# cloudflare/flow-pipeline

Measured on AMD Instinct MI355X. Metric: FlowMessages/sec aggregated into flows_5m, higher is better.
Workload: dtype u64

## Files before the change

### flow-pipeline_amd/csrc/agg.cuh

```cuda
#pragma once
#include <hip/hip_runtime.h>
#include <stdint.h>

#include "sinks.cuh"

namespace fa {

struct AggTable {
    unsigned long long k0[AGG_SLOTS], k1[AGG_SLOTS], s1[AGG_SLOTS], s2[AGG_SLOTS];
};
static_assert(sizeof(AggTable) == 32 * AGG_SLOTS, "agg_kernel LDS table");

__device__ __forceinline__ bool agg_lds_upsert(AggTable& lt, uint64_t k0, uint64_t k1, uint32_t h, uint32_t by,
                                               unsigned long long v2) {
    uint32_t i = h & (AGG_SLOTS - 1);
#pragma unroll 1
    for (int probe = 0; probe < AGG_PROBES; probe++, i = (i + 1) & (AGG_SLOTS - 1)) {
        unsigned long long c0 = lt.k0[i];
        if (c0 == 0) c0 = atomicCAS(&lt.k0[i], 0ull, (unsigned long long)k0);
        if (c0 != 0 && c0 != k0) continue;
        unsigned long long c1 = lt.k1[i];
        if (c1 == 0) c1 = atomicCAS(&lt.k1[i], 0ull, (unsigned long long)k1);
        if (c1 != 0 && c1 != k1) continue;
        if (by) atomicAdd(&lt.s1[i], (unsigned long long)by);
// ... 101 lines not shown
            if (qn + cnt > 64u) {
                agg_drain(a, lt, tb_base, lane, queue, qn);
                qn = 0;
            }
            if (pnd)
                queue[qn + (uint32_t)__builtin_popcountll(m & ((1ull << lane) - 1ull))] =
                    tup16_pack(tv[s].src_as, tv[s].dst_as, tv[s].bytes, tv[s].packets, tv[s].tbr, tv[s].etype);
            qn += cnt;
        }
    }
}

__device__ __forceinline__ void agg_consume(const KArgs& a, AggTable& lt, uint32_t tb_base, uint32_t lane, const AggBatch& b, uint4* queue,
                                            uint32_t& qn) {
    constexpr int NT = AGG_SU;
    static_assert(NT % AGG_CH == 0, "batch = whole chunks");
    agg_consume_chunk<0>(a, lt, tb_base, lane, b, queue, qn);
    if constexpr (NT > AGG_CH) agg_consume_chunk<AGG_CH>(a, lt, tb_base, lane, b, queue, qn);
    if constexpr (NT > 2 * AGG_CH) agg_consume_chunk<2 * AGG_CH>(a, lt, tb_base, lane, b, queue, qn);
    if constexpr (NT > 3 * AGG_CH) agg_consume_chunk<3 * AGG_CH>(a, lt, tb_base, lane, b, queue, qn);
    static_assert(NT <= 4 * AGG_CH, "agg_consume: add chunks");
}

__global__ __launch_bounds__(AGG_BLOCK) void agg_kernel(KArgs a) {
    __shared__ AggTable lt;
    __shared__ uint32_t pc[AGG_MAX_NWG + AGG_PAD];
    const uint32_t part = blockIdx.x;
    for (int i = threadIdx.x; i < AGG_SLOTS; i += AGG_BLOCK) {
        lt.k0[i] = 0;
        lt.k1[i] = 0;
        lt.s1[i] = 0;
        lt.s2[i] = 0;
    }
    __shared__ uint32_t pcb[AGG_MAX_NWG + AGG_PAD];
    __shared__ uint4 queues[(AGG_BLOCK / 64) * 64];
    __shared__ uint32_t maxc_s[2];
    if (threadIdx.x < 3) maxc_s[threadIdx.x] = 0;
    __syncthreads();
    uint32_t mymax = 0, mymaxb = 0, mysum = 0;
    for (uint32_t i = threadIdx.x; i < AGG_MAX_NWG + AGG_PAD; i += AGG_BLOCK) {
        const uint32_t c = i < a.nwg ? a.seg_counts[(size_t)part * a.nwg + i] : 0u;
        const uint32_t cb = i < a.nwg ? a.seg_counts[((size_t)NPART_MAX + part) * a.nwg + i] : 0u;
        pc[i] = c;
        pcb[i] = cb;
        mymax = max(mymax, c);
        mymaxb = max(mymaxb, cb);
        mysum += c + cb;
    }
    for (int o = 32; o > 0; o >>= 1) {
        mymax = max(mymax, (uint32_t)__shfl_xor((int)mymax, o));
        mymaxb = max(mymaxb, (uint32_t)__shfl_xor((int)mymaxb, o));
        mysum += (uint32_t)__shfl_xor((int)mysum, o);
    }
    if ((threadIdx.x & 63) == 0) {
        atomicMax(&maxc_s[0], mymax);
        atomicMax(&maxc_s[1], mymaxb);
        if (mysum) atomicAdd(&maxc_s[2], mysum);
    }
    const uint32_t tb_base = a.ctr->tb_base;
// ... 42 lines not shown
    ulonglong2 home[NF];
    uint32_t fh[NF];
#pragma unroll
    for (int q = 0; q < NF; q++) {
        const int i = q * AGG_BLOCK + threadIdx.x;
        fk0[q] = lt.k0[i];
        fk1[q] = lt.k1[i];
        fs1[q] = lt.s1[i];
        fs2[q] = lt.s2[i];
        fh[q] = key_hash(fk0[q], fk1[q]);
        home[q] = *reinterpret_cast<const ulonglong2*>(&a.tab[as_home(fk0[q], fk1[q], fh[q], a.mask, a.rlog2)]);
    }
#pragma unroll
    for (int q = 0; q < NF; q++) {
        Slot* sp = nullptr;
        const unsigned long long b = fs1[q], p = fs2[q] >> 25, c = fs2[q] & 0x1ffffffull;
        if (fk0[q] != 0 && fk1[q] != 0 && fs2[q] != 0) {
            if (home[q].x == fk0[q] && home[q].y == fk1[q]) sp = &a.tab[as_home(fk0[q], fk1[q], fh[q], a.mask, a.rlog2)];
            else sp = table_find_or_claim(a, fk0[q], fk1[q], fh[q]);
            if (!sp) spill_park(a, fk0[q], fk1[q], b, p, c);
        }
        quad_atomic_update(sp, b, p, c);
    }
}

constexpr int AGG8_SLOTS = 4096;
constexpr int AGG8_ALL = AGG8_SLOTS + AGG_PROBES;
struct Agg8Table {
    unsigned long long key[AGG8_ALL], s1[AGG8_ALL], s2[AGG8_ALL];
};
__device__ __forceinline__ unsigned long long agg8_key(const uint2& t) { return (1ull << 63) | ((unsigned long long)(t.y >> 26) << 32) | t.x; }
__device__ __forceinline__ uint32_t agg8_mix(const uint2& t) { return (t.x ^ ((t.y >> 26) * 0x9E3779B1u)) * 0x85EBCA6Bu; }
__device__ __forceinline__ uint32_t agg8_home(const uint2& t) {
    return agg8_mix(t) >> 20;
}
__device__ __forceinline__ uint32_t agg8_sub(const uint2& t) { return (agg8_mix(t) >> 17) & 7u; }
__device__ __forceinline__ void agg8_global(const KArgs& a, uint32_t tb_base, uint32_t part, const uint2& t, uint32_t by, uint32_t pk) {
    TupleVals v;
    t8_unpack(t, part, tb_base, v);
    uint64_t k0, k1;
    pack_key(tb_base + v.tbr, v.src_as, v.dst_as, v.etype, k0, k1);
    agg_global(a, k0, k1, key_hash(k0, k1), by, pk, 1);
}
__device__ __forceinline__ void agg8_tuple(const KArgs& a, Agg8Table& lt, uint32_t tb_base, uint32_t part, const uint2& t) {
    const unsigned long long key = agg8_key(t);
    const uint32_t by = t.y & 0x1ffffu, pk = (t.y >> 17) & 0x1ffu;
// ... 68 lines not shown
        b.v |= valid << (2 * s);
        idx[s] = valid ? piece : 0u;
    }
#pragma unroll
    for (int s = 0; s < SU; s++) b.t[s] = pbase[(size_t)min(seg[s], nwg - 1u) * (capq / 2u) + idx[s]];
}
__device__ __forceinline__ void agg8_drain(const KArgs& a, Agg8Table& lt, uint32_t tb_base, uint32_t part, uint32_t lane, const uint2* queue, uint32_t qn) {
    if (lane < qn) agg8_tuple(a, lt, tb_base, part, queue[lane]);
}
__device__ __forceinline__ unsigned long long agg8_find_heavy(unsigned long long key, bool valid) {
    unsigned long long rest = __builtin_amdgcn_ballot_w64(valid);
#pragma unroll 1
    for (int attempt = 0; attempt < 2 && rest != 0ull; attempt++) {
        const int l = __builtin_ctzll(rest);
        const unsigned long long k = readlane_u64(key, l);
        const unsigned long long same = __builtin_amdgcn_ballot_w64(valid && key == k);
        if (__builtin_popcountll(same) >= 8) return k;
        rest &= ~same;
    }
    return 0ull;
}
__device__ __forceinline__ void agg8_consume(const KArgs& a, Agg8Table& lt, uint32_t tb_base, uint32_t part, uint32_t lane, const Agg8Batch& b,
                                             uint2* queue, uint32_t& qn, uint32_t pmask, uint32_t pass, unsigned long long& hk) {
    uint2 t[AGG8_NT];
    unsigned long long key[AGG8_NT], c0[AGG8_NT], c1[AGG8_NT];
    uint32_t home[AGG8_NT];
#pragma unroll
    for (int e = 0; e < AGG8_NT; e++) {
        const uint4& q = b.t[e >> 1];
        t[e] = (e & 1) ? make_uint2(q.z, q.w) : make_uint2(q.x, q.y);
        key[e] = agg8_key(t[e]);
        home[e] = agg8_home(t[e]);
        c0[e] = lt.key[home[e]];
        c1[e] = lt.key[home[e] + 1];
    }
    if (FA_DBG(a, DBG_AGG_NO_LDS)) {
        unsigned long long x = 0;
#pragma unroll
        for (int e = 0; e < AGG8_NT; e++) x ^= c0[e] ^ c1[e] ^ key[e];
        if (x == 0x12345678ull) lt.s1[lane] = x;
        return;
    }
    uint32_t pending = 0;
    if (hk < 4ull) {
        const unsigned long long f = agg8_find_heavy(key[0], (b.v & 1u) && !(pmask && (agg8_sub(t[0]) & pmask) != pass));
        hk = f ? f : hk + 1ull;
// ... 109 lines not shown
            while (g < ngroups && j >= (uint32_t)__builtin_amdgcn_readfirstlane((int)LV[min(g, (uint32_t)(NG) - 1u)])) { \
                g += WAVES;                                                                                 \
                j = 0;                                                                                      \
            }                                                                                               \
        };                                                                                                  \
        settle_item();                                                                                      \
        Agg8Batch b0, b1;                                                                                   \
        agg8_fetch<BACK, AGG8_SU>(a.capq, a.nwg, pbase, PCNT, g * (GSEGS), lane, j, b0);                                          \
        while (g < ngroups) {                                                                               \
            j++;                                                                                            \
            settle_item();                                                                                  \
            agg8_fetch<BACK, AGG8_SU>(a.capq, a.nwg, pbase, PCNT, g * (GSEGS), lane, j, b1);                                      \
            agg8_consume(a, lt, tb_base, part, lane, b0, queue, qn, pmask, pass, hk);                                       \
            if (g >= ngroups) break;                                                                        \
            j++;                                                                                            \
            settle_item();                                                                                  \
            agg8_fetch<BACK, AGG8_SU>(a.capq, a.nwg, pbase, PCNT, g * (GSEGS), lane, j, b0);                                      \
            agg8_consume(a, lt, tb_base, part, lane, b1, queue, qn, pmask, pass, hk);                                       \
        }                                                                                                   \
    }
    FA_AGG8_PASS(false, flv, NFG, FGRP, pc)
    FA_AGG8_PASS(true, blv, NBG, BGRP, pcb)
#undef FA_AGG8_PASS
    agg8_drain(a, lt, tb_base, part, lane, queue, qn);
    __syncthreads();
    const unsigned long long tm1 = (FA_DBG(a, DBG_TIMING | DBG_AGG8_TIMING)) ? (FA_DBG(a, DBG_AGG8_TIMING) ? wall_clock64() : clock64()) : 0ull;
    if (FA_DBG(a, DBG_AGG_NO_FLUSH)) return;
    constexpr int NF = (AGG8_ALL + AGG_BLOCK - 1) / AGG_BLOCK, FB = 3;
    auto group_of = [&](int i, uint64_t& k0, uint64_t& k1, unsigned long long& s1, unsigned long long& s2) -> bool {
        const unsigned long long key = i < AGG8_ALL ? lt.key[i] : 0ull;
        s1 = i < AGG8_ALL ? lt.s1[i] : 0ull;
        s2 = i < AGG8_ALL ? lt.s2[i] : 0ull;
        TupleVals v;
        t8_unpack(make_uint2((uint32_t)key, (uint32_t)(key >> 32) << 26), part, tb_base, v);
        pack_key(tb_base + v.tbr, v.src_as, v.dst_as, v.etype, k0, k1);
        return key != 0ull && s2 != 0ull;
    };
    if (a.rlog2 == AS_RLOG2_MAX && !(a.dbg & DBG_AGG_ATOMIC_FLUSH)) {
        const uint32_t rmask = a.mask >> AS_RLOG2_MAX;
#pragma unroll 1
        for (int q0 = 0; q0 < NF; q0 += FB) {
            uint64_t fk0[FB], fk1[FB];
            unsigned long long fs1[FB], fs2[FB], cnt[FB];
            ulonglong2 kk[FB], vv[FB];
            Slot* hs[FB];
            bool valid[FB];
// ... 95 lines not shown
    }
    if (pass + 1 < npass) {
        __syncthreads();
        for (int i = threadIdx.x; i < AGG8_ALL; i += AGG_BLOCK) {
            lt.key[i] = 0;
            lt.s1[i] = 0;
            lt.s2[i] = 0;
        }
        __syncthreads();
    }
    }
    const uint32_t gw = (uint32_t)wave_sum_u64(my_groups), cw = (uint32_t)wave_sum_u64(my_created);
    __syncthreads();
    if (threadIdx.x == 0) pc[0] = pc[1] = 0;
    __syncthreads();
    if (lane == 0 && gw) atomicAdd(&pc[0], gw);
    if (lane == 0 && cw) atomicAdd(&pc[1], cw);
    __syncthreads();
    if (threadIdx.x == 0) {
        if (pc[1]) atomicAdd(&a.ctr->used, (unsigned long long)pc[1]);
        if (pc[0]) atomicAdd(&a.ctr->agg_groups, (unsigned long long)pc[0]);
        if (blockIdx.x == 0) atomicAdd(&a.ctr->agg_launches, 1ull);
    }
}

constexpr int CMS_PAD = CMS_SU * 8;
struct CmsBatch {
    uint4 t[CMS_SU];
    uint32_t v;
};
template <bool BACK>
__device__ __forceinline__ void cms_fetch(const KArgs& a, const uint4* pbase, const uint32_t* pc, uint32_t w0, uint32_t lane, uint32_t j, CmsBatch& b) {
    constexpr uint32_t SEGS = BACK ? 8u : 1u, PER = 64u / SEGS;
    uint32_t idx[CMS_SU], seg[CMS_SU];
    b.v = 0;
#pragma unroll
    for (int s = 0; s < CMS_SU; s++) {
        seg[s] = w0 + (uint32_t)s * SEGS + (BACK ? lane / PER : 0u);
        const uint32_t c = pc[min(seg[s], (uint32_t)(AGG_MAX_NWG + CMS_PAD - 1))];
        const uint32_t first = BACK ? a.capq - c : 0u;
        const uint32_t piece = first + PER * j + (BACK ? lane % PER : lane);
        const uint32_t valid = piece < first + c ? 1u : 0u;
        b.v |= valid << s;
        idx[s] = valid ? piece : 0u;
    }
#pragma unroll
// ... 210 lines not shown
```

### flow-pipeline_amd/csrc/flowagg.hip

```cpp
#include <hip/hip_runtime.h>
#include <sched.h>
#include <hipcub/hipcub.hpp>

#include <algorithm>
#include <atomic>
#include <thread>
#include <chrono>
#include <cmath>
#include <condition_variable>
#include <functional>
#include <cstdio>
#include <cstdlib>
#include <cstring>
#include <ctime>
#include <memory>
#include <mutex>
#include <string>
#include <vector>

#include "../../include/flowagg.h"
#include "kernels.cuh"

using namespace fa;

static thread_local std::string g_create_error;

struct fa_ctx {
    fa_config cfg{};
    uint32_t gran = 300;
    hipStream_t stream = nullptr;
    struct LaunchEvents { hipEvent_t e0, e1, e2; };
    std::vector<LaunchEvents> ev_pool;
    size_t ev_used = 0;
    std::vector<LaunchEvents> dev_pool;
    size_t dev_used = 0;

    Slot* tab = nullptr;
    uint32_t cap_log2 = 20;
    SpillEntry* spill = nullptr;
    uint32_t spill_cap = 0;
    Counters* d_ctr = nullptr;
    Counters* h_ctr = nullptr;
    static constexpr int NSNAP = 8;
    Counters* h_snap = nullptr;
    hipEvent_t snap_ev[NSNAP] = {};
    uint64_t snap_records[NSNAP] = {};
    uint64_t snap_seq[NSNAP] = {};
    uint64_t launch_seq = 0, known_seq = 0;
    uint64_t launched_records = 0, known_records = 0;
    Counters known{};
    uint32_t* d_exotic = nullptr;
    size_t exotic_cap = 0;
    uint4* seg = nullptr;
    size_t seg_bytes = 0;
    uint32_t* seg_counts = nullptr;
    size_t seg_counts_cap = 0;
    uint4* cseg = nullptr;
    size_t cseg_bytes = 0;
    uint32_t* cseg_counts = nullptr;
    size_t cseg_counts_cap = 0;
    HotSeed* hot_seed = nullptr;
    uint32_t* hot_seed_tag = nullptr;
    uint32_t hot_seed_wgs = 0, hot_epoch = 0;
    uint32_t cms_par = 0;
    uint32_t* cms_psize = nullptr;
    uint4* wseg = nullptr;
    size_t wseg_bytes = 0;
// ... 235 lines not shown
        return FA_ERR_ARG;
    }
    fa_ctx* c = new fa_ctx();
    c->cfg = cfg;
    c->gran = gran;
    c->cap_log2 = cfg.table_capacity_log2;
    if (const char* d = getenv("FA_DEBUG_FLAGS")) c->dbg = (uint32_t)strtoul(d, nullptr, 0);
    if (const char* d = getenv("FA_PLOG2")) c->plog2 = std::min<uint32_t>(PART_LOG2_MAX, std::max<uint32_t>(4, (uint32_t)atoi(d)));
    if (const char* d = getenv("FA_WGPC")) c->wgpc_cap = (uint32_t)atoi(d);
    if (const char* d = getenv("FA_SEG_CAP")) c->seg_cap_limit = std::max<uint32_t>(40u, (uint32_t)atoi(d) & ~7u);
    if (const char* d = getenv("FA_SINK")) c->sink_mode = !strcmp(d, "direct") ? 1 : !strcmp(d, "scatter") ? 2 : 0;
    if (const char* d = getenv("FA_CMS")) c->cms_atomic = !strcmp(d, "atomic");
    if (const char* d = getenv("FA_WIDE")) c->wide_mode = !strcmp(d, "atomic") ? 1 : !strcmp(d, "scatter") ? 2 : !strcmp(d, "log") ? 3 : 0;
    if (const char* d = getenv("FA_WIDE_LOG_CHUNKS")) c->wlog_max = (size_t)std::max(0, atoi(d));
    if (const char* d = getenv("FA_WSEG_BUDGET")) c->wseg_budget = (uint32_t)std::max(1, atoi(d));
    if (const char* d = getenv("FA_AGG_PASSES")) {
        const int v = atoi(d);
        c->agg_passes_forced = (v == 1 || v == 2 || v == 4 || v == 8) ? (uint32_t)v : 0u;
    }
    c->cms_scatter_ok = cms_scatterable(cfg.cms_depth, cfg.cms_width_log2);
    if (const char* d = getenv("FA_STAGE_THREADS")) c->stage_threads = (unsigned)std::min(64, std::max(1, atoi(d)));
    c->stage_threads = std::min(c->stage_threads, std::max(1u, std::thread::hardware_concurrency()));
    if (const char* d = getenv("FA_TUPLE")) c->t8_mode = !strcmp(d, "8") ? 1 : !strcmp(d, "16") ? 2 : 0;
    if (const char* d = getenv("FA_SEQ")) c->seq_mode = !strcmp(d, "1") ? 1 : !strcmp(d, "0") ? 2 : 0;
    auto bail = [&](const char* what, hipError_t e) {
        g_create_error = std::string("fa_create: ") + what + ": " + hipGetErrorString(e);
        fa_destroy(c);
        return e == hipErrorOutOfMemory ? FA_ERR_NOMEM : FA_ERR_HIP;
    };
    hipError_t e;
    if ((e = hipSetDevice(cfg.device)) != hipSuccess) return bail("hipSetDevice", e);
    {
        int v = 0;
        if (hipDeviceGetAttribute(&v, hipDeviceAttributeMultiprocessorCount, cfg.device) == hipSuccess && v > 0)
            c->num_cus = v;
    }
    if ((e = hipStreamCreateWithFlags(&c->stream, hipStreamNonBlocking)) != hipSuccess)
        return bail("hipStreamCreate", e);
    for (int i = 0; i < 2; i++)
        if ((e = hipEventCreateWithFlags(&c->stage_ev[i], hipEventDisableTiming)) != hipSuccess ||
            (e = hipEventCreateWithFlags(&c->copy_ev[i], hipEventDisableTiming)) != hipSuccess)
            return bail("hipEventCreate", e);
    for (int i = 0; i < fa_ctx::NSNAP; i++)
        if ((e = hipEventCreateWithFlags(&c->snap_ev[i], hipEventDisableTiming)) != hipSuccess) return bail("hipEventCreate", e);
    if ((e = hipHostMalloc(&c->h_snap, sizeof(Counters) * fa_ctx::NSNAP)) != hipSuccess) return bail("hipHostMalloc", e);
    c->spill_cap = 2u * cfg.max_batch_records + (1u << 21);
    c->wide_per_record = ((cfg.key_sets & FA_KEYS_ADDR_PORT_PROTO) ? 1u : 0u) + ((cfg.key_sets & FA_KEYS_PORT_HIST) ? 2u : 0u) +
                         ((cfg.key_sets & FA_KEYS_MINUTE_SERIES) ? 1u : 0u);
    c->wspill_cap = (uint32_t)std::min<uint64_t>((uint64_t)c->wide_per_record * 2u * cfg.max_batch_records + (1u << 21), 1u << 25);
    size_t tab_bytes = sizeof(Slot) << c->cap_log2;
    if ((e = hipMalloc(&c->tab, tab_bytes)) != hipSuccess) return bail("hipMalloc(table)", e);
    if ((e = hipMemsetAsync(c->tab, 0, tab_bytes, c->stream)) != hipSuccess) return bail("memset", e);
    if ((e = hipMalloc(&c->spill, sizeof(SpillEntry) * c->spill_cap)) != hipSuccess)
        return bail("hipMalloc(spill)", e);
    if ((e = hipMalloc(&c->d_ctr, sizeof(Counters))) != hipSuccess) return bail("hipMalloc(ctr)", e);
    if ((e = hipMemsetAsync(c->d_ctr, 0, sizeof(Counters), c->stream)) != hipSuccess)
        return bail("memset", e);
    if ((e = hipHostMalloc(&c->h_ctr, sizeof(Counters))) != hipSuccess) return bail("hipHostMalloc", e);
    if (cfg.key_sets & (FA_KEYS_SRCADDR_CMS | FA_KEYS_DSTADDR_CMS)) {
        c->cms_words = (size_t)cfg.cms_depth << cfg.cms_width_log2;
        if (cfg.key_sets & FA_KEYS_SRCADDR_CMS) {
            if ((e = hipMalloc(&c->cms_src, c->cms_words * 8 * CMS_REPLICAS)) != hipSuccess) return bail("hipMalloc(cms)", e);
            if ((e = hipMemsetAsync(c->cms_src, 0, c->cms_words * 8 * CMS_REPLICAS, c->stream)) != hipSuccess)
                return bail("memset", e);
        }
        if (cfg.key_sets & FA_KEYS_DSTADDR_CMS) {
            if ((e = hipMalloc(&c->cms_dst, c->cms_words * 8 * CMS_REPLICAS)) != hipSuccess) return bail("hipMalloc(cms)", e);
            if ((e = hipMemsetAsync(c->cms_dst, 0, c->cms_words * 8 * CMS_REPLICAS, c->stream)) != hipSuccess)
// ... 96 lines not shown
        const size_t np = (size_t)CMS_SETS * CMS_NPART;
        std::vector<uint32_t> cnt(np * c->last_nwg * 2);
        if (hipMemcpy(cnt.data(), c->cseg_counts, cnt.size() * 4, hipMemcpyDeviceToHost) == hipSuccess) {
            unsigned long long tot = 0, mx = 0, mxseg = 0;
            for (size_t p = 0; p < np; p++) {
                unsigned long long s = 0;
                for (uint32_t w = 0; w < c->last_nwg; w++) {
                    const unsigned long long v = (unsigned long long)cnt[p * c->last_nwg + w] + cnt[(np + p) * c->last_nwg + w];
                    s += v;
                    mxseg = std::max(mxseg, v);
                }
                tot += s;
                mx = std::max(mx, s);
            }
            fprintf(stderr, "[flowagg] last launch's sketch tuples: %llu, per partition mean %.0f max %llu (%.2fx), longest segment %llu (mean %.1f)\n", tot,
                    (double)tot / (double)np, mx, (double)mx * (double)np / (double)std::max(1ull, tot), mxseg, (double)tot / (double)(np * c->last_nwg));
        }
    }
    (void)hipFree(c->tab);
    (void)hipFree(c->spill);
    (void)hipFree(c->d_ctr);
    if (c->h_ctr) (void)hipHostFree(c->h_ctr);
    if (c->h_snap) (void)hipHostFree(c->h_snap);
    for (int i = 0; i < fa_ctx::NSNAP; i++)
        if (c->snap_ev[i]) (void)hipEventDestroy(c->snap_ev[i]);
    (void)hipFree(c->d_exotic);
    (void)hipFree(c->seg);
    (void)hipFree(c->seg_counts);
    (void)hipFree(c->cseg);
    (void)hipFree(c->cseg_counts);
    (void)hipFree(c->cms_psize);
    (void)hipFree(c->hot_seed);
    (void)hipFree(c->hot_seed_tag);
    (void)hipFree(c->wseg);
    (void)hipFree(c->wseg_counts);
    for (auto* v : {&c->wlog, &c->wlog_free})
        for (auto& k : *v) {
            (void)hipFree(k.seg);
            (void)hipFree(k.counts);
        }
    for (int i = 0; i < 2; i++) {
        if (c->h_stage[i]) (void)hipHostFree(c->h_stage[i]);
        (void)hipFree(c->d_in[i]);
        if (c->stage_ev[i]) (void)hipEventDestroy(c->stage_ev[i]);
        if (c->copy_ev[i]) (void)hipEventDestroy(c->copy_ev[i]);
    }
// ... 161 lines not shown
```

### flow-pipeline_amd/csrc/ingest.cuh

```cuda
#pragma once
#include <hip/hip_runtime.h>
#include <stdint.h>

#include "sinks.cuh"

#ifndef FA_FOLD_EVERY
#define FA_FOLD_EVERY 4
#endif
#ifndef FA_LT_KEEP
#define FA_LT_KEEP 8u
#endif
namespace fa {

struct NoHook {
    __device__ __forceinline__ void operator()() const {}
};
struct LaneTally {
    uint32_t ok = 0, direct = 0, second = 0, misfit8 = 0, late = 0;
    uint32_t tick = 0;
};
template <int MODE, uint32_t KEYSETS, uint32_t COLS, bool T8 = false, int CANDM = -1, class Hook = NoHook>
__device__ __forceinline__ void lane_work(const KArgs& a, LdsTable<LDS_SLOTS>& lt, LdsMinutes& lm, uint32_t* part_cnt, const uint32_t* tile,
                                          bool mine, uint32_t pos, uint32_t end, uint32_t rec_idx, uint32_t tb_base,
                                          LaneTally& tally, uint32_t& pmode, uint32_t& lt_seen, uint32_t& lt_hits,
// ... 784 lines not shown
        const uint32_t tb = (uint32_t)r.time_received / a.gran;
        if (tb < a.late_below) atomicAdd(&a.ctr->late, 1ull);
        if (ks_on<KEYSETS>(a, FA_KEYS_AS_PAIR)) {
            uint64_t k0, k1;
            pack_key(tb, r.src_as, r.dst_as, r.etype, k0, k1);
            agg_global(a, k0, k1, key_hash(k0, k1), r.bytes, r.packets, 1);
        }
        uint64_t w = r.bytes * r.sampling_rate;
        if (ks_on<KEYSETS>(a, FA_KEYS_SRCADDR_CMS)) {
            cms_add(a.cms_src, a.cms_depth, a.cms_wl2, a.cms_seed, r.src, w, a.cms_nrep);
            keyset_offer(a, 0u, r.src);
        }
        if (ks_on<KEYSETS>(a, FA_KEYS_DSTADDR_CMS)) {
            cms_add(a.cms_dst, a.cms_depth, a.cms_wl2, a.cms_seed, r.dst, w, a.cms_nrep);
            keyset_offer(a, 1u, r.dst);
        }
        if (KEYSETS & FA_KEYS_WIDE) wide_sink_slow<KEYSETS>(a, r, tb);
    }
}

template <int MODE, uint32_t KEYSETS>
__global__ __launch_bounds__(BLOCK) void deferred_kernel(KArgs a) {
    constexpr uint32_t COLS = MODE == MODE_DECODE ? (uint32_t)COL_ALL : cols_for_keysets<KEYSETS>();
    exotic_pass<MODE, KEYSETS>(a);
    const uint32_t cnt = a.ctr->retry_count[a.par];
    const uint32_t rounds = (cnt + gridDim.x * BLOCK - 1) / (gridDim.x * BLOCK);
    uint32_t n_ok = 0;
    for (uint32_t it = 0; it < rounds; it++) {
        const uint32_t j = (it * gridDim.x + blockIdx.x) * BLOCK + threadIdx.x;
        bool sure = false;
        Rec r;
        rec_clear(r);
        uint32_t idx = 0;
        if (j < cnt) {
            idx = a.retry_idx[j];
            uint32_t pos = a.off[idx], end = a.off[idx + 1];
            GlobalSrc src{reinterpret_cast<const uint32_t*>(a.buf)};
            sure = end >= pos && end <= a.len;
            if (sure && a.framed) {
                uint32_t pl = 0;
                sure = frame_fast(window64(src, pos), end - pos, pl);
                pos += pl;
            }
            if (sure) sure = parse_fast<COLS>(src, pos, end, r);
            if (!sure) {
                const uint32_t x0 = a.off[idx], x1 = a.off[idx + 1];
// ... 55 lines not shown
```

### flow-pipeline_amd/csrc/ingest_host.inc

```

template <int MODE>
static int launch_tiles(fa_ctx* c, KArgs& a, int grid, fa_ctx::LaunchEvents* ev = nullptr) {
    dim3 b(BLOCK);
    dim3 g(grid);
    dim3 ge(std::min(256u, (a.n + BLOCK - 1) / BLOCK));
    a.par = c->par;
    c->par ^= 1u;
    const bool wave_tiles = MODE == MODE_INGEST && a.seg != nullptr && c->use_wave_tiles;
    const bool t8 = wave_tiles && c->use_t8;
    hipStream_t dstream = c->stream;
    if (ev) (void)hipEventRecord(ev->e0, c->stream);
    const bool seq_variant = wave_tiles && c->cfg.key_sets == FA_KEYS_AS_PAIR && c->seq_mode != 2 && (c->seq_mode == 1 || c->stats.batches < c->seq_until);
    if (seq_variant) c->stats.learnt_order_launches += 1;
    if (wave_tiles) c->stats.wave_tile_launches += 1;
    if (t8) c->stats.compact_tuple_launches += 1;
    if (MODE == MODE_INGEST && wave_tiles && a.wseg) HIPCHK(c, hipMemsetAsync(&c->d_ctr->wtb_min, 0xff, 2 * sizeof(unsigned int), c->stream));
#define FA_LAUNCH_W(KS)                                                                         \
    do {                                                                                        \
        if constexpr ((KS & 6u) != 0u && KS != KS_ALL) {   \
            if (a.cseg) {                                                      \
                if (c->cand_state) {                                                            \
                    if (t8) hipLaunchKernelGGL((wtile_kernel<KS, true, false, 1>), g, dim3(wtile_block<KS>()), 0, c->stream, a); \
                    else hipLaunchKernelGGL((wtile_kernel<KS, false, false, 1>), g, dim3(wtile_block<KS>()), 0, c->stream, a);   \
                } else {                                                                        \
                    if (t8) hipLaunchKernelGGL((wtile_kernel<KS, true, false, 0>), g, dim3(wtile_block<KS>()), 0, c->stream, a); \
                    else hipLaunchKernelGGL((wtile_kernel<KS, false, false, 0>), g, dim3(wtile_block<KS>()), 0, c->stream, a);   \
                }                                                                               \
                break;                                                                          \
            }                                                                                   \
        }                                                                                       \
        if constexpr (KS == 1u) {                                                               \
            if (seq_variant) {                                                                  \
                if (t8) hipLaunchKernelGGL((wtile_kernel<1u, true, true>), g, dim3(wtile_block<1u>()), 0, c->stream, a); \
                else hipLaunchKernelGGL((wtile_kernel<1u, false, true>), g, dim3(wtile_block<1u>()), 0, c->stream, a);   \
                break;                                                                          \
            }                                                                                   \
        }                                                                                       \
        if (t8) hipLaunchKernelGGL((wtile_kernel<KS, true>), g, dim3(wtile_block<KS>()), 0, c->stream, a); \
        else hipLaunchKernelGGL((wtile_kernel<KS, false>), g, dim3(wtile_block<KS>()), 0, c->stream, a);   \
    } while (0)
#define FA_LAUNCH(KS)                                                                           \
    case KS: {                                                                                  \
        if constexpr (MODE == MODE_INGEST && (KS & FA_KEYS_AS_PAIR) != 0u) {                    \
            if (wave_tiles) FA_LAUNCH_W(KS);                                                    \
            else hipLaunchKernelGGL((tile_kernel<MODE, KS>), g, b, 0, c->stream, a);            \
        } else {  \
            hipLaunchKernelGGL((tile_kernel<MODE, KS>), g, b, 0, c->stream, a);                 \
        }                                                                                       \
        if (ev) (void)hipEventRecord(ev->e1, c->stream);                                        \
        hipLaunchKernelGGL((deferred_kernel<MODE, KS>), ge, b, 0, dstream, a);                  \
        break;                                                                                  \
    }
    if constexpr (MODE == MODE_DECODE) {
        switch (1u) { FA_LAUNCH(1u) }
    } else {
        switch (c->cfg.key_sets) {
            FA_LAUNCH(1u) FA_LAUNCH(2u) FA_LAUNCH(3u) FA_LAUNCH(4u) FA_LAUNCH(5u) FA_LAUNCH(6u) FA_LAUNCH(7u) FA_LAUNCH(9u)
        default:
            if (wave_tiles) FA_LAUNCH_W(KS_ALL);
            else hipLaunchKernelGGL((tile_kernel<MODE, KS_ALL>), g, b, 0, c->stream, a);
            if (ev) (void)hipEventRecord(ev->e1, c->stream);
            hipLaunchKernelGGL((deferred_kernel<MODE, KS_ALL>), ge, b, 0, dstream, a);
            break;
        }
    }
#undef FA_LAUNCH
#undef FA_LAUNCH_W
    const bool side = MODE == MODE_INGEST && wave_tiles && a.cseg && c->cand_stream && c->cand_state;
    hipStream_t agg_stream = c->stream;
    if (side) {
        HIPCHK(c, hipEventRecord(c->cand_ev[0], c->stream));
        HIPCHK(c, hipStreamWaitEvent(c->cand_stream, c->cand_ev[0], 0));
        agg_stream = c->cand_stream;
    }
    if (MODE == MODE_INGEST && a.seg) {
        const dim3 ga(1u << a.plog2);
        if (t8) hipLaunchKernelGGL(agg8_kernel, ga, dim3(AGG_BLOCK), 0, agg_stream, a);
        else hipLaunchKernelGGL(agg_kernel, ga, dim3(AGG_BLOCK), 0, agg_stream, a);
    }
    const hipError_t side_done = side ? hipEventRecord(c->cand_ev[1], c->cand_stream) : hipSuccess;
    const int rc = [&]() -> int {
        if (MODE == MODE_INGEST && wave_tiles && a.cseg) {
            const uint32_t set_mask = (c->cfg.key_sets >> 1) & 3u;
            const uint32_t nlog = CMS_NPART * (set_mask == 3u ? 2u : 1u);
// ... 3 lines not shown
        if (MODE == MODE_INGEST && c->cand_state) {
            HIPCHK(c, hipMemsetAsync(c->cand_state, 0, 2 * sizeof(CandState), c->stream));
            const dim3 gs(CAND_SCAN_BLOCKS, 2), gb(256, 2);
            hipLaunchKernelGGL(cand_scan_kernel, gs, dim3(256), 0, c->stream, c->ks_src, c->ks_dst, 1u << c->ks_log2, (const unsigned long long*)c->cms_src,
                               (const unsigned long long*)c->cms_dst, c->cfg.cms_depth, c->cfg.cms_width_log2, c->cfg.cms_seed, c->cand_state, c->cand_chunkmax);
            hipLaunchKernelGGL(cand_bits_kernel, gb, dim3(256), 0, c->stream, (const KeySlot*)c->ks_src, (const KeySlot*)c->ks_dst, (const unsigned long long*)c->cms_src,
                               (const unsigned long long*)c->cms_dst, c->cfg.cms_depth, c->cfg.cms_width_log2, c->cfg.topk_track, std::max(c->ks_log2, 8u) - 2u, c->cand_state,
                               c->cand_bits[0], c->cand_bits[1]);
        }
        if (MODE == MODE_INGEST && wave_tiles && a.wseg) {
            if (c->wlog_now) {
                HIPCHK(c, hipMemcpyAsync(c->wseg_counts + c->wseg_counts_cap, &c->d_ctr->tb_base, 3 * sizeof(uint32_t), hipMemcpyDeviceToDevice, c->stream));
            } else {
                hipLaunchKernelGGL(wagg_kernel, dim3(1u << a.wplog2), dim3(WAGG_BLOCK), 0, c->stream, a, (const uint32_t*)nullptr, 0u);
            }
        }
        return FA_OK;
    }();
    if (side && (side_done != hipSuccess || hipStreamWaitEvent(c->stream, c->cand_ev[1], 0) != hipSuccess)) {
        (void)hipStreamSynchronize(c->cand_stream);
        if (rc == FA_OK) return fail(c, FA_ERR_HIP, "joining the side stream failed");
    }
    if (rc) return rc;
    if (ev) (void)hipEventRecord(ev->e2, c->stream);
    HIPCHK(c, hipGetLastError());
    return FA_OK;
}

template <int MODE>
static int tile_grid(fa_ctx* c, uint32_t n, uint32_t tile_recs) {
    if constexpr (MODE == MODE_DECODE) return grid_for(c, tile_kernel<MODE_DECODE, 1u>, n, tile_recs);
    switch (c->cfg.key_sets) {
    case 1u: return grid_for(c, tile_kernel<MODE_INGEST, 1u>, n, tile_recs);
    case 2u: return grid_for(c, tile_kernel<MODE_INGEST, 2u>, n, tile_recs);
    case 3u: return grid_for(c, tile_kernel<MODE_INGEST, 3u>, n, tile_recs);
    case 4u: return grid_for(c, tile_kernel<MODE_INGEST, 4u>, n, tile_recs);
    case 5u: return grid_for(c, tile_kernel<MODE_INGEST, 5u>, n, tile_recs);
    case 6u: return grid_for(c, tile_kernel<MODE_INGEST, 6u>, n, tile_recs);
    case 7u: return grid_for(c, tile_kernel<MODE_INGEST, 7u>, n, tile_recs);
    case 9u: return grid_for(c, tile_kernel<MODE_INGEST, 9u>, n, tile_recs);
    default: return grid_for(c, tile_kernel<MODE_INGEST, KS_ALL>, n, tile_recs);
    }
}

static int ensure_exotic(fa_ctx* c, size_t n) {
    if (c->exotic_cap >= n) return FA_OK;
    HIPCHK(c, hipStreamSynchronize(c->stream));
// ... 310 lines not shown
        if (n > lim) {
            for (size_t i = 0; i < n; i += lim) {
                const size_t m = std::min(lim, n - i);
                int rc1 = ingest_device_records(c, d_buf, len, (size_t)((double)bytes * (double)m / (double)n), (const uint32_t*)d_off + i, m);
                if (rc1) return rc1;
            }
            return FA_OK;
        }
    }
    const bool scatter = (c->cfg.key_sets & FA_KEYS_AS_PAIR) && (c->sink_mode == 2 || (c->sink_mode == 0 && n >= (1u << 15)));
    c->use_wave_tiles = scatter;
    c->use_t8 = c->use_wave_tiles && c->plog2 == 8 && c->t8_mode != 2 && (c->t8_mode == 1 || c->stats.batches >= c->t8_wide_until);
    if (n > AGG_MAX_BATCH && !c->use_t8) {
        const size_t h = n / 2;
        int rc1 = ingest_device_records(c, d_buf, len, bytes / 2, d_off, h);
        if (rc1) return rc1;
        return ingest_device_records(c, d_buf, len, bytes - bytes / 2, (const uint32_t*)d_off + h, n - h);
    }
    int rc = pre_launch_guard(c, n);
    if (rc) return rc;
    rc = ensure_exotic(c, n);
    if (rc) return rc;
    if (c->ev_used == c->ev_pool.size()) {
        if (c->ev_pool.size() >= 4096) {
            rc = settle(c);
            if (rc) return rc;
        } else {
            fa_ctx::LaunchEvents e{};
            HIPCHK(c, hipEventCreate(&e.e0));
            HIPCHK(c, hipEventCreate(&e.e1));
            HIPCHK(c, hipEventCreate(&e.e2));
            c->ev_pool.push_back(e);
        }
    }
    KArgs a = make_args(c);
    a.buf = (const uint8_t*)d_buf;
    a.off = (const uint32_t*)d_off;
    a.n = (uint32_t)n;
    a.len = (uint32_t)len;
    a.tile_recs = tile_recs_for(bytes, n);
    int grid = tile_grid<MODE_INGEST>(c, a.n, a.tile_recs);
    if (c->use_wave_tiles) {
        const double avg = (double)bytes / (double)n;
        const bool big_wg = !wt_lean(c->cfg.key_sets);
        const uint32_t ks = c->cfg.key_sets;
        auto recs_for = [&](double cap) {
            double r = cap / avg;
// ... 259 lines not shown
```

### flow-pipeline_amd/csrc/maintain_host.inc

```

static int rebuild_table(fa_ctx* c, uint32_t new_log2, uint32_t tb_lo, uint32_t tb_hi) {
    Slot* nt = nullptr;
    size_t bytes = sizeof(Slot) << new_log2;
    hipError_t e = hipMalloc(&nt, bytes);
    if (e != hipSuccess) return fail(c, FA_ERR_NOMEM, "rebuild_table: hipMalloc failed");
    if ((e = hipMemsetAsync(nt, 0, bytes, c->stream)) != hipSuccess ||
        (e = hipMemsetAsync(&c->d_ctr->used, 0, sizeof(unsigned long long), c->stream)) != hipSuccess) {
        (void)hipFree(nt);
        c->err = std::string("rebuild_table: ") + hipGetErrorString(e);
        return FA_ERR_HIP;
    }
    Slot* old = c->tab;
    uint32_t old_slots = 1u << c->cap_log2;
    c->tab = nt;
    c->cap_log2 = new_log2;
    KArgs a = make_args(c);
    hipLaunchKernelGGL(rebuild_kernel, dim3(1024), dim3(256), 0, c->stream, old, old_slots, tb_lo, tb_hi, a);
    HIPCHK(c, hipGetLastError());
    HIPCHK(c, hipStreamSynchronize(c->stream));
    HIPCHK(c, hipFree(old));
    c->used_base = 0;
    c->stats.table_capacity = 1ull << c->cap_log2;
    return FA_OK;
}
// ... 106 lines not shown
            c->seen_wused = h.wused;
            c->seen_wfold = h.wfold_n;
        }
    }
    if (h.agg_launches < c->seen_agg_launches || h.agg_groups < c->seen_agg_groups) c->seen_agg_launches = c->seen_agg_groups = 0;
    const uint64_t d_l = h.agg_launches - c->seen_agg_launches, d_g = h.agg_groups - c->seen_agg_groups;
    if (d_l) {
        const uint64_t per_part = d_g / d_l >> c->plog2;
        uint32_t want = 1;
        while (want < 8 && per_part > (uint64_t)(AGG8_SLOTS / 2) * want) want *= 2;
        if (want > c->agg_passes) c->agg_passes = std::min(want, c->agg_passes * 2);
        else if (want < c->agg_passes && per_part * 3 < (uint64_t)(AGG8_SLOTS / 2) * c->agg_passes) c->agg_passes = std::max(want, c->agg_passes / 2);
        c->seen_agg_launches = h.agg_launches;
        c->seen_agg_groups = h.agg_groups;
    }
}

static int settle(fa_ctx* c) {
    if (c->cms_dirty) {
        int frc = cms_fold(c);
        if (frc) return frc;
    }
    HIPCHK(c, hipMemcpyAsync(c->h_ctr, c->d_ctr, sizeof(Counters), hipMemcpyDeviceToHost, c->stream));
    HIPCHK(c, hipStreamSynchronize(c->stream));
    for (size_t i = 0; i < c->ev_used; i++) {
        float ms = 0;
        if (hipEventElapsedTime(&ms, c->ev_pool[i].e0, c->ev_pool[i].e1) == hipSuccess) {
            c->stats.kernel_ns = (uint64_t)((double)ms * 1e6);
            c->stats.kernel_ns_total += c->stats.kernel_ns;
            c->stats.kernel_launches += 1;
        }
        if (hipEventElapsedTime(&ms, c->ev_pool[i].e0, c->ev_pool[i].e2) == hipSuccess)
            c->stats.batch_ns_total += (uint64_t)((double)ms * 1e6);
    }
    c->ev_used = 0;
    for (size_t i = 0; i < c->dev_used; i++) {
        float ms = 0;
        if (hipEventElapsedTime(&ms, c->dev_pool[i].e0, c->dev_pool[i].e2) == hipSuccess) {
            c->stats.decode_ns_total += (uint64_t)((double)ms * 1e6);
            c->stats.decode_launches += 1;
        }
    }
    c->dev_used = 0;
    Counters h = *c->h_ctr;
    c->stats.records_ok = h.ok;
    c->stats.records_bad = h.bad;
    c->stats.records_slow = h.slow;
    c->stats.records_direct = h.direct;
    c->stats.records_retried = h.retried;
// ... 189 lines not shown
}
static int pre_launch_guard(fa_ctx* c, size_t n) {
    auto verdict = [&]() -> int {
        const Counters& h = c->known;
        if (h.spill_count || h.wspill_count || (c->used_base + h.used) * 2 > (1ull << c->cap_log2) ||
            (c->wtab && (c->wused_base + h.wused) * 2 > (1ull << c->wcap_log2)))
            return 2;
        const uint64_t pot = (c->launched_records - c->known_records) + n;
        if (pot + (1u << 20) > c->spill_cap || (c->wtab && pot * c->wide_per_record + (1u << 20) > c->wspill_cap)) return 1;
        return 0;
    };
    poll_snapshots(c, false);
    int v = verdict();
    if (v == 1) {
        poll_snapshots(c, true);
        v = verdict() ? 2 : 0;
    }
    return v == 2 ? settle(c) : FA_OK;
}
static int post_launch_snapshot(fa_ctx* c, size_t n) {
    c->launched_records += n;
    c->launch_seq += 1;
    const int k = (int)((c->launch_seq - 1) % fa_ctx::NSNAP);
    HIPCHK(c, hipEventSynchronize(c->snap_ev[k]));
    HIPCHK(c, hipMemcpyAsync(&c->h_snap[k], c->d_ctr, sizeof(Counters), hipMemcpyDeviceToHost, c->stream));
    HIPCHK(c, hipEventRecord(c->snap_ev[k], c->stream));
    c->snap_records[k] = c->launched_records;
    c->snap_seq[k] = c->launch_seq;
    c->snap_wpot[k] = c->wpot_total;
    return FA_OK;
}

extern "C" int fa_sync(fa_ctx* c) {
    FA_ON_DEVICE(c);
    if (!c) return FA_ERR_ARG;
    if (c->sticky) return c->sticky;
    return settle(c);
}
```

### flow-pipeline_amd/csrc/sinks.cuh

```cuda
#pragma once
#include <hip/hip_runtime.h>
#include <stdint.h>

#include "gen.cuh"
#include "table.cuh"
#include "wide.cuh"
#include "wire.cuh"

namespace fa {

constexpr int BLOCK = 256;
constexpr int TILE_BYTES = 21760;
constexpr int TILE_PAD = 112;
constexpr int TILE_STRIDE = TILE_BYTES + TILE_PAD;
constexpr int LDS_SLOTS = 64;
constexpr int LDS_PROBES = 2;
constexpr int PART_LOG2_MAX = 8;
constexpr int NPART_MAX = 1 << PART_LOG2_MAX;
#ifndef FA_WBLOCK
#define FA_WBLOCK 768
#endif
#ifndef FA_WT_STRIDE
#define FA_WT_STRIDE 4864
#endif
// ... 19 lines not shown
#ifndef FA_AGG_SLOTS
#define FA_AGG_SLOTS 4096
#endif
constexpr int AGG_SLOTS = FA_AGG_SLOTS;
constexpr int AGG_PROBES = 16;
constexpr uint32_t AGG_MAX_BATCH = 1u << 24;
constexpr uint32_t AGG8_MAX_BATCH = (1u << 25) - 1u;
static_assert(TILE_STRIDE % 16 == 0, "LDS tile buffers must stay 16-byte aligned");

enum { MODE_INGEST = 0, MODE_DECODE = 1 };
constexpr uint32_t KS_ALL = 0xFFu;
constexpr uint32_t FA_KEYS_WIDE = FA_KEYS_ADDR_PORT_PROTO | FA_KEYS_PORT_HIST | FA_KEYS_MINUTE_SERIES;
constexpr uint32_t PORT_DENSE = 65536;
#ifndef FA_ABLATE
#define FA_ABLATE 0
#endif
#ifndef FA_TL_WINDOW
#define FA_TL_WINDOW 256u
#endif
#define FA_DBG(a, flags) (FA_ABLATE != 0 && ((a).dbg & (flags)) != 0)
enum { DBG_NO_SINK = 1, DBG_LOOP_PARSER = 2, DBG_NO_LDS_TABLE = 4, DBG_NO_GLOBAL = 8, DBG_NO_PARSE = 16, DBG_NO_TUPLE_STORE = 32,
       DBG_AGG_NO_LDS = 64, DBG_AGG_NO_FLUSH = 128, DBG_AGG_NO_SLOW = 256, DBG_DMA_NO_NT = 512, DBG_TIMING = 1024, DBG_TUPLE_NT = 2048, DBG_TUPLE_SC = 4096, DBG_NO_LANE_OFF = 8192, DBG_SYNTH_TILES = 16384, DBG_NOT_MINE = 32768, DBG_NO_SECOND = 65536, DBG_NO_FRAME = 131072, DBG_NO_KEYSET = 262144, DBG_NO_CMS = 524288, DBG_NO_HOT = 1048576, DBG_CMS_TUPLE_LOCAL = 268435456 , DBG_NO_SINGLES = 134217728 , DBG_TUPLE_LOCAL = 67108864 , DBG_CAND_NO_SET = 33554432 , DBG_AGG_ATOMIC_FLUSH = 2097152 ,
       DBG_AGG8_TIMING = 8388608 ,
       DBG_CMS_TIMING = 4194304  };

struct SpillEntry {
    unsigned long long k0, k1, bytes, packets, count;
};

struct Counters {
    unsigned long long ok, bad, slow, spill_lost, used, direct, retried;
    unsigned long long misfit8;
    unsigned int exotic_count[2], retry_count[2];
    unsigned int spill_count, rows_count, ks_overflow, ks_rows;
    unsigned int tb_base, wtb_min, wtb_nmax, pad;
    unsigned long long t_wait, t_work, t_tiles, t_total;
    unsigned long long wfold_n;
    unsigned long long wused, wspill_lost;
    unsigned int wspill_count, wrows_count;
    unsigned long long agg_groups, agg_launches;
    unsigned long long late;
};

struct __attribute__((aligned(32))) KeySlot {
    unsigned long long tag, lo, hi, pad;
};
constexpr unsigned long long KS_CLAIMED = 1ull << 63, KS_READY = 1ull << 62;
struct TopkRow {
    unsigned long long lo, hi, weight;
};
constexpr uint32_t TK_BINS = 2048;
__host__ __device__ __forceinline__ uint32_t topk_bin(unsigned long long est) {
    if (est < 64ull) return (uint32_t)est;
#if defined(__HIP_DEVICE_COMPILE__)
    const uint32_t e = 63u - (uint32_t)__clzll((long long)est);
#else
    const uint32_t e = 63u - (uint32_t)__builtin_clzll(est);
#endif
    return ((e - 4u) << 5) | ((uint32_t)(est >> (e - 5u)) & 31u);
}
__host__ __device__ __forceinline__ unsigned long long topk_bin_floor(uint32_t b) {
    if (b < 64u) return b;
    const uint32_t e = (b >> 5) + 4u;
    return (1ull << e) | ((unsigned long long)(b & 31u) << (e - 5u));
// ... 53 lines not shown
    uint32_t rlog2;
    uint32_t agg_passes;
    uint4* cseg;
    uint32_t* cseg_counts;
    uint32_t ccapq, ccapf, ccapb;
    unsigned long long cregion;
    uint32_t cms_sub;
    HotSeed* hot_seed;
    uint32_t* hot_seed_tag;
    uint32_t hot_epoch;
    uint32_t* cms_psize;
    uint32_t key_sets;
    WSlot* wtab;
    uint32_t wmask;
    WSpillEntry* wspill;
    uint32_t wspill_cap;
    uint4* wseg;
    uint32_t* wseg_counts;
    uint32_t wcapq;
    uint32_t wplog2;
    unsigned long long wregion;
    ulonglong2* port_hist;
    uint32_t late_below;
};

__device__ __forceinline__ KArgs cold_args() {
#if defined(__HIP_DEVICE_COMPILE__)
    const KArgs* p = (const KArgs*)__builtin_amdgcn_kernarg_segment_ptr();
    asm volatile("" : "+s"(p));
    return *p;
#else
    return KArgs{};
#endif
}

__device__ __forceinline__ WArgs wargs(const KArgs& a) {
    return WArgs{a.wtab, a.wmask, a.wmask >> a.wplog2, a.wspill, a.wspill_cap, &a.ctr->wspill_count, &a.ctr->wspill_lost, &a.ctr->wused};
}
template <uint32_t KEYSETS>
__device__ __forceinline__ bool ks_on(const KArgs& a, uint32_t x) {
    return (KEYSETS & x) != 0 && (KEYSETS != KS_ALL || (a.key_sets & x) != 0);
}

__device__ __forceinline__ void agg_global(const KArgs& a, uint64_t k0, uint64_t k1, uint32_t h,
                                           uint64_t b, uint64_t p, uint64_t c) {
    uint32_t i = as_home(k0, k1, h, a.mask, a.rlog2);
// ... 669 lines not shown
```

Measured before the change: 48.68 billion.

## Publish counter snapshot from last agg block and replace timing events with device stamps

```diff
diff --git a/flow-pipeline_amd/csrc/agg.cuh b/flow-pipeline_amd/csrc/agg.cuh
--- a/flow-pipeline_amd/csrc/agg.cuh
+++ b/flow-pipeline_amd/csrc/agg.cuh
@@ -147,6 +147,30 @@
     static_assert(NT <= 4 * AGG_CH, "agg_consume: add chunks");
 }
 
+__global__ void stamp_kernel(unsigned long long* p) { *p = wall_clock64(); }
+__device__ __forceinline__ void publish_snapshot(const KArgs& a, uint32_t* lds_flag) {
+    if (a.snap == nullptr) return;
+    __builtin_amdgcn_s_waitcnt(0);
+    __syncthreads();
+    if (threadIdx.x == 0) {
+        const unsigned int t = __hip_atomic_fetch_add(&a.ctr->snap_ticket, 1u, __ATOMIC_RELAXED, __HIP_MEMORY_SCOPE_AGENT);
+        *lds_flag = t + 1u == gridDim.x ? 1u : 0u;
+    }
+    __syncthreads();
+    if (*lds_flag == 0u) return;
+    constexpr uint32_t WORDS = sizeof(Counters) / sizeof(uint32_t), TICKET = offsetof(Counters, snap_ticket) / sizeof(uint32_t);
+    static_assert(sizeof(Counters) % sizeof(uint32_t) == 0 && WORDS <= 64u, "one wave copies the counters, a word per lane");
+    if (threadIdx.x < WORDS) {
+        uint32_t v = __hip_atomic_load(reinterpret_cast<const uint32_t*>(a.ctr) + threadIdx.x, __ATOMIC_RELAXED, __HIP_MEMORY_SCOPE_AGENT);
+        if (threadIdx.x == TICKET) v = 0u;
+        __hip_atomic_store(reinterpret_cast<uint32_t*>(a.snap) + threadIdx.x, v, __ATOMIC_RELAXED, __HIP_MEMORY_SCOPE_SYSTEM);
+    }
+    if (threadIdx.x == 0) {
+        __hip_atomic_store(&a.ctr->snap_ticket, 0u, __ATOMIC_RELAXED, __HIP_MEMORY_SCOPE_AGENT);
+        if (a.stamps) a.stamps[2] = wall_clock64();
+    }
+}
+
 __global__ __launch_bounds__(AGG_BLOCK) void agg_kernel(KArgs a) {
     __shared__ AggTable lt;
     __shared__ uint32_t pc[AGG_MAX_NWG + AGG_PAD];
@@ -159,7 +183,7 @@
     }
     __shared__ uint32_t pcb[AGG_MAX_NWG + AGG_PAD];
     __shared__ uint4 queues[(AGG_BLOCK / 64) * 64];
-    __shared__ uint32_t maxc_s[2];
+    __shared__ uint32_t maxc_s[3];
     if (threadIdx.x < 3) maxc_s[threadIdx.x] = 0;
     __syncthreads();
     uint32_t mymax = 0, mymaxb = 0, mysum = 0;
@@ -248,6 +272,7 @@
         }
         quad_atomic_update(sp, b, p, c);
     }
+    publish_snapshot(a, &maxc_s[0]);
 }
 
 constexpr int AGG8_SLOTS = 4096;
@@ -362,6 +387,13 @@
 }
 __device__ __forceinline__ void agg8_consume(const KArgs& a, Agg8Table& lt, uint32_t tb_base, uint32_t part, uint32_t lane, const Agg8Batch& b,
                                              uint2* queue, uint32_t& qn, uint32_t pmask, uint32_t pass, unsigned long long& hk) {
+    if (FA_DBG(a, DBG_AGG_WALK_ONLY)) {
+        unsigned long long x = b.v;
+#pragma unroll
+        for (int s = 0; s < AGG8_SU; s++) x ^= ((unsigned long long)(b.t[s].x ^ b.t[s].z) << 32) | (b.t[s].y ^ b.t[s].w);
+        hk ^= x;
+        return;
+    }
     uint2 t[AGG8_NT];
     unsigned long long key[AGG8_NT], c0[AGG8_NT], c1[AGG8_NT];
     uint32_t home[AGG8_NT];
@@ -517,6 +549,10 @@
     FA_AGG8_PASS(false, flv, NFG, FGRP, pc)
     FA_AGG8_PASS(true, blv, NBG, BGRP, pcb)
 #undef FA_AGG8_PASS
+    if (FA_DBG(a, DBG_AGG_WALK_ONLY)) {
+        if (hk == 0x12345678ull) lt.s1[lane] = hk;
+        qn = 0;
+    }
     agg8_drain(a, lt, tb_base, part, lane, queue, qn);
     __syncthreads();
     const unsigned long long tm1 = (FA_DBG(a, DBG_TIMING | DBG_AGG8_TIMING)) ? (FA_DBG(a, DBG_AGG8_TIMING) ? wall_clock64() : clock64()) : 0ull;
@@ -658,6 +694,7 @@
         if (pc[0]) atomicAdd(&a.ctr->agg_groups, (unsigned long long)pc[0]);
         if (blockIdx.x == 0) atomicAdd(&a.ctr->agg_launches, 1ull);
     }
+    publish_snapshot(a, &pc[2]);
 }
 
 constexpr int CMS_PAD = CMS_SU * 8;
diff --git a/flow-pipeline_amd/csrc/flowagg.hip b/flow-pipeline_amd/csrc/flowagg.hip
--- a/flow-pipeline_amd/csrc/flowagg.hip
+++ b/flow-pipeline_amd/csrc/flowagg.hip
@@ -29,7 +29,10 @@
     fa_config cfg{};
     uint32_t gran = 300;
     hipStream_t stream = nullptr;
-    struct LaunchEvents { hipEvent_t e0, e1, e2; };
+    struct LaunchEvents {
+        hipEvent_t e0, e1, e2;
+        bool stamped;
+    };
     std::vector<LaunchEvents> ev_pool;
     size_t ev_used = 0;
     std::vector<LaunchEvents> dev_pool;
@@ -43,6 +46,14 @@
     Counters* h_ctr = nullptr;
     static constexpr int NSNAP = 8;
     Counters* h_snap = nullptr;
+    Counters* d_snap = nullptr;
+    bool snap_copy = false;
+    bool snap_in_kernel = false;
+    static constexpr size_t EV_POOL_MAX = 4096;
+    unsigned long long* d_stamps = nullptr;
+    unsigned long long* h_stamps = nullptr;
+    bool stamped_launches = false;
+    double stamp_ns = 10.0;
     hipEvent_t snap_ev[NSNAP] = {};
     uint64_t snap_records[NSNAP] = {};
     uint64_t snap_seq[NSNAP] = {};
@@ -324,6 +335,7 @@
     if (const char* d = getenv("FA_STAGE_THREADS")) c->stage_threads = (unsigned)std::min(64, std::max(1, atoi(d)));
     c->stage_threads = std::min(c->stage_threads, std::max(1u, std::thread::hardware_concurrency()));
     if (const char* d = getenv("FA_TUPLE")) c->t8_mode = !strcmp(d, "8") ? 1 : !strcmp(d, "16") ? 2 : 0;
+    if (const char* d = getenv("FA_SNAP")) c->snap_copy = !strcmp(d, "copy");
     if (const char* d = getenv("FA_SEQ")) c->seq_mode = !strcmp(d, "1") ? 1 : !strcmp(d, "0") ? 2 : 0;
     auto bail = [&](const char* what, hipError_t e) {
         g_create_error = std::string("fa_create: ") + what + ": " + hipGetErrorString(e);
@@ -346,6 +358,13 @@
     for (int i = 0; i < fa_ctx::NSNAP; i++)
         if ((e = hipEventCreateWithFlags(&c->snap_ev[i], hipEventDisableTiming)) != hipSuccess) return bail("hipEventCreate", e);
     if ((e = hipHostMalloc(&c->h_snap, sizeof(Counters) * fa_ctx::NSNAP)) != hipSuccess) return bail("hipHostMalloc", e);
+    if ((e = hipHostGetDevicePointer((void**)&c->d_snap, c->h_snap, 0)) != hipSuccess) return bail("hipHostGetDevicePointer", e);
+    if ((e = hipHostMalloc(&c->h_stamps, sizeof(unsigned long long) * 4 * fa_ctx::EV_POOL_MAX)) != hipSuccess) return bail("hipHostMalloc", e);
+    if ((e = hipMalloc(&c->d_stamps, sizeof(unsigned long long) * 4 * fa_ctx::EV_POOL_MAX)) != hipSuccess) return bail("hipMalloc(stamps)", e);
+    {
+        int khz = 0;
+        if (hipDeviceGetAttribute(&khz, hipDeviceAttributeWallClockRate, cfg.device) == hipSuccess && khz > 0) c->stamp_ns = 1e6 / (double)khz;
+    }
     c->spill_cap = 2u * cfg.max_batch_records + (1u << 21);
     c->wide_per_record = ((cfg.key_sets & FA_KEYS_ADDR_PORT_PROTO) ? 1u : 0u) + ((cfg.key_sets & FA_KEYS_PORT_HIST) ? 2u : 0u) +
                          ((cfg.key_sets & FA_KEYS_MINUTE_SERIES) ? 1u : 0u);
@@ -488,6 +507,8 @@
     (void)hipFree(c->d_ctr);
     if (c->h_ctr) (void)hipHostFree(c->h_ctr);
     if (c->h_snap) (void)hipHostFree(c->h_snap);
+    if (c->h_stamps) (void)hipHostFree(c->h_stamps);
+    (void)hipFree(c->d_stamps);
     for (int i = 0; i < fa_ctx::NSNAP; i++)
         if (c->snap_ev[i]) (void)hipEventDestroy(c->snap_ev[i]);
     (void)hipFree(c->d_exotic);
diff --git a/flow-pipeline_amd/csrc/ingest.cuh b/flow-pipeline_amd/csrc/ingest.cuh
--- a/flow-pipeline_amd/csrc/ingest.cuh
+++ b/flow-pipeline_amd/csrc/ingest.cuh
@@ -830,6 +830,7 @@
 template <int MODE, uint32_t KEYSETS>
 __global__ __launch_bounds__(BLOCK) void deferred_kernel(KArgs a) {
     constexpr uint32_t COLS = MODE == MODE_DECODE ? (uint32_t)COL_ALL : cols_for_keysets<KEYSETS>();
+    if (a.stamps && blockIdx.x == 0 && threadIdx.x == 0) a.stamps[1] = wall_clock64();
     exotic_pass<MODE, KEYSETS>(a);
     const uint32_t cnt = a.ctr->retry_count[a.par];
     const uint32_t rounds = (cnt + gridDim.x * BLOCK - 1) / (gridDim.x * BLOCK);
diff --git a/flow-pipeline_amd/csrc/ingest_host.inc b/flow-pipeline_amd/csrc/ingest_host.inc
--- a/flow-pipeline_amd/csrc/ingest_host.inc
+++ b/flow-pipeline_amd/csrc/ingest_host.inc
@@ -9,7 +9,21 @@
     const bool wave_tiles = MODE == MODE_INGEST && a.seg != nullptr && c->use_wave_tiles;
     const bool t8 = wave_tiles && c->use_t8;
     hipStream_t dstream = c->stream;
-    if (ev) (void)hipEventRecord(ev->e0, c->stream);
+    c->snap_in_kernel = MODE == MODE_INGEST && a.seg != nullptr && !c->snap_copy && c->dbg == 0 && !a.cseg && !a.wseg && !c->cand_state && !c->wtab;
+    if (ev) ev->stamped = false;
+    if (c->snap_in_kernel) {
+        const int k = (int)(c->launch_seq % fa_ctx::NSNAP);
+        HIPCHK(c, hipEventSynchronize(c->snap_ev[k]));
+        a.snap = &c->d_snap[k];
+        const size_t slot = ev ? (size_t)(ev - c->ev_pool.data()) : fa_ctx::EV_POOL_MAX;
+        if (slot < fa_ctx::EV_POOL_MAX) {
+            a.stamps = c->d_stamps + 4 * slot;
+            ev->stamped = true;
+            c->stamped_launches = true;
+            hipLaunchKernelGGL(stamp_kernel, dim3(1), dim3(1), 0, c->stream, a.stamps);
+        }
+    }
+    if (ev && !a.stamps) (void)hipEventRecord(ev->e0, c->stream);
     const bool seq_variant = wave_tiles && c->cfg.key_sets == FA_KEYS_AS_PAIR && c->seq_mode != 2 && (c->seq_mode == 1 || c->stats.batches < c->seq_until);
     if (seq_variant) c->stats.learnt_order_launches += 1;
     if (wave_tiles) c->stats.wave_tile_launches += 1;
@@ -47,7 +61,7 @@
         } else {  \
             hipLaunchKernelGGL((tile_kernel<MODE, KS>), g, b, 0, c->stream, a);                 \
         }                                                                                       \
-        if (ev) (void)hipEventRecord(ev->e1, c->stream);                                        \
+        if (ev && !a.stamps) (void)hipEventRecord(ev->e1, c->stream);                                        \
         hipLaunchKernelGGL((deferred_kernel<MODE, KS>), ge, b, 0, dstream, a);                  \
         break;                                                                                  \
     }
@@ -59,7 +73,7 @@
         default:
             if (wave_tiles) FA_LAUNCH_W(KS_ALL);
             else hipLaunchKernelGGL((tile_kernel<MODE, KS_ALL>), g, b, 0, c->stream, a);
-            if (ev) (void)hipEventRecord(ev->e1, c->stream);
+            if (ev && !a.stamps) (void)hipEventRecord(ev->e1, c->stream);
             hipLaunchKernelGGL((deferred_kernel<MODE, KS_ALL>), ge, b, 0, dstream, a);
             break;
         }
@@ -109,7 +123,7 @@
         if (rc == FA_OK) return fail(c, FA_ERR_HIP, "joining the side stream failed");
     }
     if (rc) return rc;
-    if (ev) (void)hipEventRecord(ev->e2, c->stream);
+    if (ev && !a.stamps) (void)hipEventRecord(ev->e2, c->stream);
     HIPCHK(c, hipGetLastError());
     return FA_OK;
 }
@@ -466,7 +480,7 @@
     rc = ensure_exotic(c, n);
     if (rc) return rc;
     if (c->ev_used == c->ev_pool.size()) {
-        if (c->ev_pool.size() >= 4096) {
+        if (c->ev_pool.size() >= fa_ctx::EV_POOL_MAX) {
             rc = settle(c);
             if (rc) return rc;
         } else {
diff --git a/flow-pipeline_amd/csrc/maintain_host.inc b/flow-pipeline_amd/csrc/maintain_host.inc
--- a/flow-pipeline_amd/csrc/maintain_host.inc
+++ b/flow-pipeline_amd/csrc/maintain_host.inc
@@ -152,9 +152,22 @@
         if (frc) return frc;
     }
     HIPCHK(c, hipMemcpyAsync(c->h_ctr, c->d_ctr, sizeof(Counters), hipMemcpyDeviceToHost, c->stream));
+    if (c->stamped_launches)
+        HIPCHK(c, hipMemcpyAsync(c->h_stamps, c->d_stamps, sizeof(unsigned long long) * 4 * std::min(c->ev_used, (size_t)fa_ctx::EV_POOL_MAX), hipMemcpyDeviceToHost, c->stream));
+    c->stamped_launches = false;
     HIPCHK(c, hipStreamSynchronize(c->stream));
     for (size_t i = 0; i < c->ev_used; i++) {
         float ms = 0;
+        if (c->ev_pool[i].stamped) {
+            const unsigned long long* t = c->h_stamps + 4 * i;
+            if (t[1] >= t[0] && t[2] >= t[1]) {
+                c->stats.kernel_ns = (uint64_t)((double)(t[1] - t[0]) * c->stamp_ns);
+                c->stats.kernel_ns_total += c->stats.kernel_ns;
+                c->stats.kernel_launches += 1;
+                c->stats.batch_ns_total += (uint64_t)((double)(t[2] - t[0]) * c->stamp_ns);
+            }
+            continue;
+        }
         if (hipEventElapsedTime(&ms, c->ev_pool[i].e0, c->ev_pool[i].e1) == hipSuccess) {
             c->stats.kernel_ns = (uint64_t)((double)ms * 1e6);
             c->stats.kernel_ns_total += c->stats.kernel_ns;
@@ -390,8 +403,11 @@
     c->launched_records += n;
     c->launch_seq += 1;
     const int k = (int)((c->launch_seq - 1) % fa_ctx::NSNAP);
-    HIPCHK(c, hipEventSynchronize(c->snap_ev[k]));
-    HIPCHK(c, hipMemcpyAsync(&c->h_snap[k], c->d_ctr, sizeof(Counters), hipMemcpyDeviceToHost, c->stream));
+    if (!c->snap_in_kernel) {
+        HIPCHK(c, hipEventSynchronize(c->snap_ev[k]));
+        HIPCHK(c, hipMemcpyAsync(&c->h_snap[k], c->d_ctr, sizeof(Counters), hipMemcpyDeviceToHost, c->stream));
+    }
+    c->snap_in_kernel = false;
     HIPCHK(c, hipEventRecord(c->snap_ev[k], c->stream));
     c->snap_records[k] = c->launched_records;
     c->snap_seq[k] = c->launch_seq;
diff --git a/flow-pipeline_amd/csrc/sinks.cuh b/flow-pipeline_amd/csrc/sinks.cuh
--- a/flow-pipeline_amd/csrc/sinks.cuh
+++ b/flow-pipeline_amd/csrc/sinks.cuh
@@ -65,6 +65,7 @@
 enum { DBG_NO_SINK = 1, DBG_LOOP_PARSER = 2, DBG_NO_LDS_TABLE = 4, DBG_NO_GLOBAL = 8, DBG_NO_PARSE = 16, DBG_NO_TUPLE_STORE = 32,
        DBG_AGG_NO_LDS = 64, DBG_AGG_NO_FLUSH = 128, DBG_AGG_NO_SLOW = 256, DBG_DMA_NO_NT = 512, DBG_TIMING = 1024, DBG_TUPLE_NT = 2048, DBG_TUPLE_SC = 4096, DBG_NO_LANE_OFF = 8192, DBG_SYNTH_TILES = 16384, DBG_NOT_MINE = 32768, DBG_NO_SECOND = 65536, DBG_NO_FRAME = 131072, DBG_NO_KEYSET = 262144, DBG_NO_CMS = 524288, DBG_NO_HOT = 1048576, DBG_CMS_TUPLE_LOCAL = 268435456 , DBG_NO_SINGLES = 134217728 , DBG_TUPLE_LOCAL = 67108864 , DBG_CAND_NO_SET = 33554432 , DBG_AGG_ATOMIC_FLUSH = 2097152 ,
        DBG_AGG8_TIMING = 8388608 ,
+       DBG_AGG_WALK_ONLY = 16777216 ,
        DBG_CMS_TIMING = 4194304  };
 
 struct SpillEntry {
@@ -83,6 +84,7 @@
     unsigned int wspill_count, wrows_count;
     unsigned long long agg_groups, agg_launches;
     unsigned long long late;
+    unsigned int snap_ticket, snap_pad;
 };
 
 struct __attribute__((aligned(32))) KeySlot {
@@ -182,6 +184,8 @@
     unsigned long long wregion;
     ulonglong2* port_hist;
     uint32_t late_below;
+    Counters* snap;
+    unsigned long long* stamps;
 };
 
 __device__ __forceinline__ KArgs cold_args() {
```

After: 49.50 billion (median of 6 runs). About the same (+1.7%).
